# ashvardanian/StringWars

Hardware: AMD Instinct MI355X
Metric: GCUPS (DP cell updates/s) batched Levenshtein (higher is better)
Workload: dtype u32; 1 GPU; C2 tokens64: 1000000 ASCII token pairs per GPU, lengths U[32,96], unbounded Levenshtein, tapes prepared and resident in HBM; step=one synchronous call (results visible on return), pairs_per_gpu=1000000, pairs_total=1000000, cells_per_gpu=4273938131, algorithm=auto, offsets=uint32, collective=none, seed=42

## Files before the change

stringwars_amd/csrc/bp_item.hpp:

```cpp
#pragma once
#include <type_traits>

#include "common.hpp"
#include "bp_window.hpp"

namespace swh {

struct SymWindow32 {
    const uint32_t *base;
    int lo, hi;
    __device__ __forceinline__ void init(const uint32_t *data, uint64_t start, uint64_t total) {
        auto c31 = [](int64_t v) { return (int)(v < -0x40000000ll ? -0x40000000ll : (v > 0x40000000ll ? 0x40000000ll : v)); };
        base = data + start;
        lo = c31(-(int64_t)start);
        hi = c31((int64_t)total - (int64_t)start - 1);
    }
    __device__ __forceinline__ uint32_t fetch(int idx) const { return base[bp_med3i(idx, lo, hi)]; }
    __device__ __forceinline__ void fetch4(int idx, uint32_t (&out)[4]) const {
        if (hi - lo >= 3) {
            const int c = bp_med3i(idx, lo, hi - 3);
            uint4 v;
            __builtin_memcpy(&v, base + c, 16);
            out[0] = v.x; out[1] = v.y; out[2] = v.z; out[3] = v.w;
            if (__builtin_expect(c == idx, 1)) return;
        }
#pragma unroll
        for (int q = 0; q < 4; ++q) out[q] = fetch(idx + q);
    }
};

template <typename Sym> struct BpTraits;
template <> struct BpTraits<uint8_t> {
    static constexpr int kWaves = 4, kEntries = 32, kMinWavesPerSimd = 4;
};
template <> struct BpTraits<uint32_t> {
    static constexpr int kWaves = 2, kEntries = 56, kMinWavesPerSimd = 2;
};
template <typename Sym> constexpr int bp_table_words() { return BpTraits<Sym>::kEntries * 64; }
template <typename Sym> constexpr size_t bp_lds_bytes() {
    return (size_t)BpTraits<Sym>::kWaves * (bp_table_words<Sym>() + 64) * 4 + 80 * 4;
}

struct GroupTables3 {
    uint32_t tbase, mask;
    __device__ __forceinline__ void init(uint32_t *table, int lane) {
        tbase = (uint32_t)(uintptr_t)(lds_u32 *)(table + lane);
        if (tbase & 0x700u) __builtin_trap();
        mask = 0x700u;
        asm volatile("" : "+v"(mask));
    }
    template <int G> __device__ __forceinline__ uint32_t addr(uint32_t c) const {
        uint32_t s;
        if constexpr (3 * G <= 8) s = c << (8 - 3 * G);
        else s = c >> (3 * G - 8);
        return (uint32_t)__builtin_amdgcn_bitop3_b32((int)s, (int)mask, (int)tbase, 0xEA);
    }
    __device__ __forceinline__ uint32_t lookup(uint32_t c) const { return lookup_n<7>(c); }
    __device__ __forceinline__ void insert(uint32_t c, uint32_t bit) const { insert_n<7>(c, bit); }
    template <int NG, int G> __device__ __forceinline__ uint32_t entry_n(uint32_t c) const {
        if constexpr (G + 1 == NG && NG < 7) {
            uint32_t idx = c >> (3 * G);
            idx = idx < 8u ? idx : 8u;
            return *(const lds_u32 *)(uintptr_t)(tbase + (idx << 8) + 2048u * G);
        } else {
            return *(const lds_u32 *)(uintptr_t)(addr<G>(c) + 2048u * G);
        }
    }
    template <int NG> __device__ __forceinline__ uint32_t lookup_n(uint32_t c) const {
        uint32_t e = entry_n<NG, 0>(c) & entry_n<NG, 1>(c);
        e &= entry_n<NG, 2>(c) & entry_n<NG, 3>(c);
        if constexpr (NG > 4) e &= entry_n<NG, 4>(c);
        if constexpr (NG > 5) e &= entry_n<NG, 5>(c);
        if constexpr (NG > 6) e &= entry_n<NG, 6>(c);
        return e;
    }
    template <int NG> __device__ __forceinline__ void insert_n(uint32_t c, uint32_t bit) const {
        __hip_atomic_fetch_or((lds_u32 *)(uintptr_t)addr<0>(c), bit, __ATOMIC_RELAXED, __HIP_MEMORY_SCOPE_WORKGROUP);
        __hip_atomic_fetch_or((lds_u32 *)(uintptr_t)(addr<1>(c) + 2048), bit, __ATOMIC_RELAXED, __HIP_MEMORY_SCOPE_WORKGROUP);
        __hip_atomic_fetch_or((lds_u32 *)(uintptr_t)(addr<2>(c) + 4096), bit, __ATOMIC_RELAXED, __HIP_MEMORY_SCOPE_WORKGROUP);
        __hip_atomic_fetch_or((lds_u32 *)(uintptr_t)(addr<3>(c) + 6144), bit, __ATOMIC_RELAXED, __HIP_MEMORY_SCOPE_WORKGROUP);
        if constexpr (NG > 4) __hip_atomic_fetch_or((lds_u32 *)(uintptr_t)(addr<4>(c) + 8192), bit, __ATOMIC_RELAXED, __HIP_MEMORY_SCOPE_WORKGROUP);
        if constexpr (NG > 5) __hip_atomic_fetch_or((lds_u32 *)(uintptr_t)(addr<5>(c) + 10240), bit, __ATOMIC_RELAXED, __HIP_MEMORY_SCOPE_WORKGROUP);
        if constexpr (NG > 6) __hip_atomic_fetch_or((lds_u32 *)(uintptr_t)(addr<6>(c) + 12288), bit, __ATOMIC_RELAXED, __HIP_MEMORY_SCOPE_WORKGROUP);
    }
};

template <typename Sym>
struct BpWave {
    static constexpr bool kBytes = sizeof(Sym) == 1;
    uint32_t *table;
    uint32_t *acc;
    NibbleTables nib;
    GroupTables3 grp;
    int lane;
    uint64_t a_total, b_total;
    __device__ __forceinline__ void init(uint32_t *table_, uint32_t *acc_, int lane_, uint64_t a_total_, uint64_t b_total_) {
        table = table_; acc = acc_; lane = lane_; a_total = a_total_; b_total = b_total_;
        if constexpr (kBytes) nib.init(table, lane);
        else grp.init(table, lane);
#pragma unroll
        for (int k = 0; k < BpTraits<Sym>::kEntries; ++k) table[k * 64 + lane] = 0;
    }
};

template <typename Sym, bool kWide>
__device__ __forceinline__ void bp_item(const KernelArgs &args, BpWave<Sym> &wv, const uint32_t G, const bool have, const uint64_t p,
                                        const uint64_t a0, const uint32_t la, const uint64_t b0, const uint32_t lb,
                                        uint16_t *staged = nullptr, const uint64_t staged_base = 0) {
    constexpr bool kBytes = sizeof(Sym) == 1;
    constexpr bool wide_tapes = kWide;
    const int lane = wv.lane;
    uint32_t *const table = wv.table;
    uint32_t *const acc = wv.acc;
    [[maybe_unused]] const NibbleTables &nib = wv.nib;
    [[maybe_unused]] const GroupTables3 &grp = wv.grp;
    const uint64_t a_total = wv.a_total, b_total = wv.b_total;
    const uint32_t slot = (uint32_t)lane / G, blk = (uint32_t)lane - slot * G;
    const bool a_is_pattern = bp_pattern_is_a(la, lb);
    const uint32_t m = a_is_pattern ? la : lb, n = a_is_pattern ? lb : la;
    using Window = typename std::conditional<kBytes, ByteWindow, SymWindow32>::type;
    Window pat, txt;
    pat.init((const Sym *)(a_is_pattern ? args.job.a.data : args.job.b.data), a_is_pattern ? a0 : b0,
             a_is_pattern ? a_total : b_total);
    txt.init((const Sym *)(a_is_pattern ? args.job.b.data : args.job.a.data), a_is_pattern ? b0 : a0,
             a_is_pattern ? b_total : a_total);

    const uint32_t row0 = blk * 32;
    const uint32_t brows = have ? (m > row0 ? (m - row0 < 32 ? m - row0 : 32) : 0) : 0;

    constexpr int kTextRegs = kBytes ? 4 : 16;
    uint32_t tnxt[kTextRegs];
    int tshift[kBytes ? 4 : 1];
    auto fetch_text = [&](int first) {
        if constexpr (kBytes) {
            if (wide_tapes) {
                tshift[0] = txt.fetch16_raw(first, tnxt);
            } else {
#pragma unroll
                for (int q = 0; q < 4; ++q) tnxt[q] = txt.fetch4_raw(first + q * 4, tshift[q]);
            }
        } else {
#pragma unroll
            for (int q = 0; q < 16; q += 4) {
                uint32_t four[4];
                txt.fetch4(first + q, four);
#pragma unroll
                for (int r = 0; r < 4; ++r) tnxt[q + r] = four[r];
            }
        }
    };
    fetch_text(0 - (int)blk);
    [[maybe_unused]] uint32_t groups = 7;

    if constexpr (kBytes) {
        uint32_t praw[8];
        int pshift[8];
        if (wide_tapes) {
            uint32_t half[2][4];
            const int moved0 = pat.fetch16_raw((int)row0, half[0]), moved1 = pat.fetch16_raw((int)row0 + 16, half[1]);
            pat.fix16((int)row0, moved0, half[0]);
            pat.fix16((int)row0 + 16, moved1, half[1]);
#pragma unroll
            for (int q = 0; q < 8; ++q) { praw[q] = half[q >> 2][q & 3]; pshift[q] = 24; }
        } else {
#pragma unroll
            for (int q = 0; q < 8; ++q) praw[q] = pat.fetch4_raw((int)row0 + q * 4, pshift[q]);
        }
        const uint32_t row_mask = brows >= 32 ? 0xFFFFFFFFu : ((1u << brows) - 1u);
#pragma unroll
        for (int q = 0; q < 8; ++q) {
            if (brows > (uint32_t)q * 4) {
                const uint32_t dw = ByteWindow::realign(praw[q], pshift[q]);
                nib.template insert<0>(dw, row_mask & (1u << (q * 4 + 0)));
                nib.template insert<1>(dw, row_mask & (1u << (q * 4 + 1)));
                nib.template insert<2>(dw, row_mask & (1u << (q * 4 + 2)));
                nib.template insert<3>(dw, row_mask & (1u << (q * 4 + 3)));
            }
        }
    } else {
        uint32_t psym[32];
#pragma unroll
        for (int q = 0; q < 32; q += 4) {
            uint32_t four[4];
            pat.fetch4((int)row0 + q, four);
#pragma unroll
            for (int r = 0; r < 4; ++r) psym[q + r] = four[r];
        }
        uint32_t seen = 0;
#pragma unroll
        for (int q = 0; q < 32; ++q) seen |= (uint32_t)q < brows ? psym[q] : 0u;
#pragma unroll
        for (int off = 32; off >= 1; off >>= 1) seen |= (uint32_t)__shfl_xor((int)seen, off);
        groups = seen < (1u << 12) ? 4u : (seen < (1u << 15) ? 5u : (seen < (1u << 18) ? 6u : 7u));
        auto enter = [&](auto ng_tag) {
            constexpr int NG = decltype(ng_tag)::value;
#pragma unroll
            for (int q = 0; q < 32; ++q)
                if ((uint32_t)q < brows) grp.template insert_n<NG>(psym[q], 1u << q);
        };
        if (groups == 4) enter(std::integral_constant<int, 4>{});
        else if (groups == 5) enter(std::integral_constant<int, 5>{});
        else if (groups == 6) enter(std::integral_constant<int, 6>{});
        else enter(std::integral_constant<int, 7>{});
    }
    acc[lane] = 0;
    wave_lds_fence();

    const uint32_t n_eff = wave_max_u32(have ? n + G - 1 : 0);
    const uint32_t steps = (n_eff + 15) & ~15u;

    const bool first_blk = blk == 0;
    uint32_t keep_mask = first_blk ? 0u : 0xFFFFFFFFu, first_ph = first_blk ? 0x80000000u : 0u;
    asm volatile("" : "+v"(keep_mask), "+v"(first_ph));
    uint32_t pv = 0xFFFFFFFFu, mv = 0, ph = 0, mh = 0;
    auto column = [&](uint32_t eq, uint32_t s) {
        uint32_t ph_in = (uint32_t)__builtin_amdgcn_update_dpp(0, (int)ph, 0x138, 0xf, 0xf, true);
        uint32_t mh_in = (uint32_t)__builtin_amdgcn_update_dpp(0, (int)mh, 0x138, 0xf, 0xf, true);
        ph_in = (uint32_t)__builtin_amdgcn_bitop3_b32((int)ph_in, (int)keep_mask, (int)first_ph, 0xEA);
        mh_in = mh_in & keep_mask;
        if (s - blk < n) {
            uint32_t xv = eq | mv;
            eq |= mh_in >> 31;
            uint32_t xh = (((eq & pv) + pv) ^ pv) | eq;
            ph = mv | ~(xh | pv);
            mh = pv & xh;
            uint32_t ph_s = __builtin_amdgcn_alignbit(ph, ph_in, 31);
            uint32_t mh_s = __builtin_amdgcn_alignbit(mh, mh_in, 31);
            pv = mh_s | ~(xv | ph_s);
            mv = ph_s & xv;
        }
    };
    auto columns = [&](auto ng_tag) {
    [[maybe_unused]] constexpr int NG = decltype(ng_tag)::value;
    for (uint32_t s0 = 0; s0 < steps; s0 += 16) {
        uint32_t tcur[kTextRegs];
        if constexpr (kBytes) {
            if (wide_tapes) {
#pragma unroll
                for (int q = 0; q < 4; ++q) tcur[q] = tnxt[q];
                txt.fix16((int)s0 - (int)blk, tshift[0], tcur);
            } else {
#pragma unroll
                for (int q = 0; q < 4; ++q) tcur[q] = ByteWindow::realign(tnxt[q], tshift[q]);
            }
        } else {
#pragma unroll
            for (int q = 0; q < kTextRegs; ++q) tcur[q] = tnxt[q];
        }
        fetch_text((int)s0 + 16 - (int)blk);
#pragma unroll
        for (int q = 0; q < 4; ++q) {
            const uint32_t gs = s0 + q * 4;
            if (gs >= n_eff) break;
            uint32_t eqs[4];
            if constexpr (kBytes) {
                eqs[0] = nib.template lookup<0>(tcur[q]);
                eqs[1] = nib.template lookup<1>(tcur[q]);
                eqs[2] = nib.template lookup<2>(tcur[q]);
                eqs[3] = nib.template lookup<3>(tcur[q]);
            } else {
#pragma unroll
                for (int u = 0; u < 4; ++u) eqs[u] = grp.template lookup_n<NG>(tcur[q * 4 + u]);
            }
#pragma unroll
            for (int u = 0; u < 4; ++u) column(eqs[u], gs + u);
        }
    }
    };
    if constexpr (kBytes) columns(std::integral_constant<int, 7>{});
    else if (groups == 4) columns(std::integral_constant<int, 4>{});
    else if (groups == 5) columns(std::integral_constant<int, 5>{});
    else if (groups == 6) columns(std::integral_constant<int, 6>{});
    else columns(std::integral_constant<int, 7>{});

    const uint32_t mask = brows >= 32 ? 0xFFFFFFFFu : ((1u << brows) - 1u);
    int part = __popc(pv & mask) - __popc(mv & mask);
    if (have && brows) atomicAdd(&acc[slot * G], (uint32_t)part);
    wave_lds_fence();
    if (have && first_blk) {
        uint32_t d = n + acc[lane];
        const uint32_t bounded = clamp_bound(d, args.job.bound);
        if (staged && bounded < 0xFFFFu) staged[p - staged_base] = (uint16_t)bounded;
        else store_result(args.job, p, (int64_t)bounded);
    }
    if constexpr (kBytes) {
#pragma unroll
        for (int k = 0; k < BpTraits<Sym>::kEntries; ++k) table[k * 64 + lane] = 0;
    } else {
#pragma unroll
        for (int k = 0; k < 32; ++k) table[k * 64 + lane] = 0;
        if (groups > 4) {
#pragma unroll
            for (int k = 32; k < BpTraits<Sym>::kEntries; ++k) table[k * 64 + lane] = 0;
        }
    }
    wave_lds_fence();
}

}
```

stringwars_amd/csrc/tiled.hip:

```cpp
#include <cstdio>
#include <cstdlib>

#include "bp_item.hpp"

namespace swh {

constexpr int tile_index_bits(int waves) { return waves >= 16 ? 12 : 11; }
constexpr int tile_max(int waves) { return 1 << tile_index_bits(waves); }
constexpr uint32_t kAffixCap = 16;
constexpr int kTileBuckets = 32;
constexpr int kTileClasses = 64;
constexpr int kTileBins = kTileClasses * kTileBuckets;

template <int kTileMax>
struct TileLds {
    uint32_t sorted[kTileMax];
    uint32_t bins[kTileBins / 2 > kTileMax / 2 ? kTileBins / 2 : kTileMax / 2];
    uint32_t class_count[kTileClasses];
    uint16_t class_thr[kTileClasses];
    uint16_t class_tgt[kTileClasses];
    uint32_t item_prefix[kTileClasses + 1];
    uint32_t wave_sums[16];
    uint32_t ticket;
};
struct TileTail {
    unsigned long long cells, syms;
    uint32_t maxa, maxb, shorts, misfit;
    SummaryLds summary;
};
static_assert(sizeof(TileTail) <= sizeof(uint32_t) * kTileBins / 2, "the tail reuses TileLds::bins");

template <typename Sym, int kWaves> constexpr size_t tiled_lds_bytes() {
    return (size_t)kWaves * (bp_table_words<Sym>() + 64) * 4 + sizeof(TileLds<tile_max(kWaves)>);
}

#ifdef SWH_TILE_PROFILE
__device__ unsigned long long g_tile_phase[8];
__device__ unsigned long long g_tile_span[2048][4];
extern "C" void swh_debug_tile_spans(unsigned long long *out) {
    (void)hipDeviceSynchronize();
    (void)hipMemcpyFromSymbol(out, HIP_SYMBOL(g_tile_span), sizeof(unsigned long long) * 2048 * 4);
}
extern "C" void swh_debug_tile_phases(unsigned long long *out) {
    unsigned long long zero[8] = {};
    (void)hipDeviceSynchronize();
    (void)hipMemcpyFromSymbol(out, HIP_SYMBOL(g_tile_phase), sizeof(zero));
    (void)hipMemcpyToSymbol(HIP_SYMBOL(g_tile_phase), zero, sizeof(zero));
}
#define TILE_STAMP(slot) do { const unsigned long long now__ = __builtin_readcyclecounter(); phase_acc[slot] += now__ - phase_t; phase_t = now__; } while (0)
#else
#define TILE_STAMP(slot) do {} while (0)
#endif

struct TiledArgs {
    KernelArgs k;
    uint32_t tile;
    uint32_t tiles;
    uint32_t shift;
    uint32_t cut_affixes;
    PlanPartial *partials;
    uint32_t *done_counter;
    CallSummary *summary;
};

template <typename Sym, int kWaves, bool kWide>
__device__ __forceinline__ void tiled_run(const TiledArgs &targs, char *smem, const uint64_t a_total, const uint64_t b_total) {
    constexpr int kThreads = kWaves * 64, kTableWords = bp_table_words<Sym>();
    constexpr int kTileMax = tile_max(kWaves), kTileIndexBits = tile_index_bits(kWaves);
    constexpr int kPer = (kTileMax + kThreads - 1) / kThreads;
    const KernelArgs &args = targs.k;
    const int lane = threadIdx.x & 63, wave = threadIdx.x >> 6;
    BpWave<Sym> wv;
    wv.init((uint32_t *)smem + (size_t)wave * kTableWords, (uint32_t *)smem + (size_t)kWaves * kTableWords + wave * 64, lane,
            a_total, b_total);
    TileLds<kTileMax> &tl = *(TileLds<kTileMax> *)(smem + (size_t)kWaves * (kTableWords + 64) * 4);
    unsigned long long cells = 0, syms = 0;
    uint32_t maxa = 0, maxb = 0, shorts = 0, misfit = 0;
#ifdef SWH_TILE_PROFILE
    unsigned long long phase_acc[4] = {0, 0, 0, 0}, phase_t = __builtin_readcyclecounter(), items_done = 0;
    if (threadIdx.x == 0) g_tile_span[blockIdx.x][0] = __builtin_amdgcn_s_memrealtime();
#endif

    for (uint32_t tile = blockIdx.x; tile < targs.tiles; tile += gridDim.x) {
        const uint64_t base = (uint64_t)tile * targs.tile;
        const uint32_t count = (uint32_t)(args.job.pairs - base < targs.tile ? args.job.pairs - base : targs.tile);
        __builtin_amdgcn_s_setprio(3);
        for (int i = threadIdx.x; i < kTileBins / 2; i += kThreads) tl.bins[i] = 0;
        if (threadIdx.x < kTileClasses) tl.class_count[threadIdx.x] = 0;
        if (threadIdx.x == 0) tl.ticket = 0;
        __syncthreads();
        uint32_t cls[kPer], txt[kPer], rank[kPer], affix[kPer];
#ifndef SWH_TILE_BATCH
#define SWH_TILE_BATCH 2
#endif
        constexpr int kBatch = kPer < SWH_TILE_BATCH ? kPer : SWH_TILE_BATCH;
        static_assert(kPer % kBatch == 0, "pairs per thread come in whole batches");
#pragma unroll
        for (int kb = 0; kb < kPer; kb += kBatch) {
        uint64_t a0s[kBatch], b0s[kBatch];
        uint32_t las[kBatch], lbs[kBatch];
#pragma unroll
        for (int j = 0; j < kBatch; ++j) {
            const int k = kb + j;
            const uint64_t p = base + (uint32_t)k * kThreads + threadIdx.x;
            const uint64_t pc = p < args.job.pairs ? p : args.job.pairs - 1;
            if (args.off64) pair_extent<uint64_t, true>(args.job, pc, a0s[j], las[j], b0s[j], lbs[j]);
            else pair_extent<uint32_t, true>(args.job, pc, a0s[j], las[j], b0s[j], lbs[j]);
            affix[k] = 0;
        }
        if constexpr (sizeof(Sym) == 1 && kWide) {
            if (targs.cut_affixes) {
                uint4 ha[kBatch], hb[kBatch], ta[kBatch], tb[kBatch];
                bool inside[kBatch];
#pragma unroll
                for (int j = 0; j < kBatch; ++j) {
                    const uint64_t ea = a0s[j] + las[j], eb = b0s[j] + lbs[j];
                    inside[j] = a0s[j] + 16 <= a_total && b0s[j] + 16 <= b_total && ea >= 16 && eb >= 16;
                    const uint8_t *ad = (const uint8_t *)args.job.a.data, *bd = (const uint8_t *)args.job.b.data;
                    __builtin_memcpy(&ha[j], ad + (inside[j] ? a0s[j] : 0), 16);
                    __builtin_memcpy(&hb[j], bd + (inside[j] ? b0s[j] : 0), 16);
                    __builtin_memcpy(&ta[j], ad + (inside[j] ? ea - 16 : 0), 16);
                    __builtin_memcpy(&tb[j], bd + (inside[j] ? eb - 16 : 0), 16);
                }
#pragma unroll
                for (int j = 0; j < kBatch; ++j) {
                    const uint32_t mn = las[j] < lbs[j] ? las[j] : lbs[j];
                    const unsigned long long h_lo = (unsigned long long)(ha[j].x ^ hb[j].x) | ((unsigned long long)(ha[j].y ^ hb[j].y) << 32);
                    const unsigned long long h_hi = (unsigned long long)(ha[j].z ^ hb[j].z) | ((unsigned long long)(ha[j].w ^ hb[j].w) << 32);
                    const unsigned long long t_lo = (unsigned long long)(ta[j].x ^ tb[j].x) | ((unsigned long long)(ta[j].y ^ tb[j].y) << 32);
                    const unsigned long long t_hi = (unsigned long long)(ta[j].z ^ tb[j].z) | ((unsigned long long)(ta[j].w ^ tb[j].w) << 32);
                    uint32_t pre = h_lo ? (uint32_t)__builtin_ctzll(h_lo) >> 3 : (h_hi ? 8u + ((uint32_t)__builtin_ctzll(h_hi) >> 3) : kAffixCap);
                    pre = pre < mn ? pre : mn;
                    uint32_t suf = t_hi ? (uint32_t)__builtin_clzll(t_hi) >> 3 : (t_lo ? 8u + ((uint32_t)__builtin_clzll(t_lo) >> 3) : kAffixCap);
                    suf = suf < mn - pre ? suf : mn - pre;
                    affix[kb + j] = inside[j] ? pre | (suf << 6) : 0u;
                }
            }
        }
#pragma unroll
        for (int j = 0; j < kBatch; ++j) {
            const int k = kb + j;
            const uint32_t idx = (uint32_t)k * kThreads + threadIdx.x;
            cls[k] = 0xFFu; txt[k] = 0; rank[k] = 0;
            if (idx < count) {
                const uint64_t p = base + idx;
                uint32_t la = las[j], lb = lbs[j];
                cells += (unsigned long long)la * lb;
                syms += (unsigned long long)la + lb;
                maxa = la > maxa ? la : maxa;
                maxb = lb > maxb ? lb : maxb;
                shorts += (la <= 32 && lb <= 32) ? 1u : 0u;
                if ((la | lb) >= kStringLimit) { misfit = 1; continue; }
                const uint32_t diff = la > lb ? la - lb : lb - la;
                const uint32_t shared = (affix[k] & 63u) + (affix[k] >> 6);
                la -= shared; lb -= shared;
                if (la == 0 || lb == 0) {
                    store_result(args.job, p, (int64_t)clamp_bound(la + lb, args.job.bound));
                } else if (args.job.bound != 0xFFFFFFFFu && diff > args.job.bound) {
                    store_result(args.job, p, (int64_t)args.job.bound + 1);
                } else {
                    const bool pattern_is_a = bp_pattern_is_a(la, lb);
                    const uint32_t m = pattern_is_a ? la : lb, n = pattern_is_a ? lb : la;
                    const uint32_t g = (m + 31) >> 5;
                    if (g > (uint32_t)kTileClasses) {
                        misfit = 1;
                    } else {
                        cls[k] = g - 1;
                        txt[k] = n;
                        rank[k] = atomicAdd(&tl.class_count[g - 1], 1u);
                    }
                }
            }
        }
        }
        __syncthreads();
        if (wave == 0) {
            const uint32_t mine = tl.class_count[lane];
            tl.class_thr[lane] = (uint16_t)mine;
            tl.class_tgt[lane] = (uint16_t)lane;
            unsigned long long present = __ballot(mine != 0);
            wave_lds_fence();
            if (lane == 0) {
                uint32_t incoming = 0;
                while (present) {
                    const int c = __builtin_ctzll(present);
                    present &= present - 1;
                    const uint32_t native = tl.class_count[c];
                    uint32_t total = native + incoming;
                    incoming = 0;
                    const uint32_t per = 64u / (uint32_t)(c + 1), rest = total % per;
                    if (rest && present) {
                        const int up = __builtin_ctzll(present);
                        const uint32_t per_up = 64u / (uint32_t)(up + 1);
                        if (rest <= native && 2 * rest <= per_up) {
                            tl.class_thr[c] = (uint16_t)(native - rest);
                            tl.class_tgt[c] = (uint16_t)up;
                            incoming = rest;
                            total -= rest;
                        }
                    }
                    tl.class_count[c] = total;
                }
            }
            wave_lds_fence();
            const uint32_t final_count = tl.class_count[lane], per = 64u / (uint32_t)(lane + 1);
            const uint32_t items = (final_count + per - 1) / per;
            const uint32_t incl = wave_inclusive_sum_u32(items);
            tl.item_prefix[lane] = incl - items;
            if (lane == 63) tl.item_prefix[64] = incl;
        }
        __syncthreads();
        uint32_t key[kPer];
#pragma unroll
        for (int k = 0; k < kPer; ++k) {
            key[k] = 0xFFFFFFFFu;
            if (cls[k] != 0xFFu) {
                uint32_t c = cls[k];
                if (rank[k] >= tl.class_thr[c]) c = tl.class_tgt[c];
                const uint32_t bucket = txt[k] >> targs.shift;
                key[k] = c * kTileBuckets + (bucket < (uint32_t)kTileBuckets - 1 ? bucket : (uint32_t)kTileBuckets - 1);
                const uint32_t old = atomicAdd(&tl.bins[key[k] >> 1], (key[k] & 1u) ? 0x10000u : 1u);
                rank[k] = (key[k] & 1u) ? old >> 16 : old & 0xFFFFu;
            }
        }
        __syncthreads();
        {
            constexpr int kWords = (kTileBins / 2 + kThreads - 1) / kThreads;
            uint32_t words[kWords], sum = 0;
#pragma unroll
            for (int q = 0; q < kWords; ++q) {
                const int at = threadIdx.x * kWords + q;
                words[q] = at < kTileBins / 2 ? tl.bins[at] : 0u;
                sum += (words[q] & 0xFFFFu) + (words[q] >> 16);
            }
            const uint32_t incl = wave_inclusive_sum_u32(sum);
            if (lane == 63) tl.wave_sums[wave] = incl;
            __syncthreads();
            uint32_t run = incl - sum;
            for (int w = 0; w < wave; ++w) run += tl.wave_sums[w];
#pragma unroll
            for (int q = 0; q < kWords; ++q) {
                const uint32_t lo = words[q] & 0xFFFFu, hi = words[q] >> 16;
                const int at = threadIdx.x * kWords + q;
                if (at < kTileBins / 2) tl.bins[at] = run | ((run + lo) << 16);
                run += lo + hi;
            }
        }
        __syncthreads();
#pragma unroll
        for (int k = 0; k < kPer; ++k) {
            if (key[k] != 0xFFFFFFFFu) {
                const uint32_t word = tl.bins[key[k] >> 1];
                const uint32_t start = (key[k] & 1u) ? word >> 16 : word & 0xFFFFu;
                tl.sorted[start + rank[k]] = ((uint32_t)k * kThreads + threadIdx.x) | (affix[k] << kTileIndexBits);
            }
        }
        __syncthreads();
        TILE_STAMP(0);
#ifdef SWH_TILE_PROFILE
        if (threadIdx.x == 0) g_tile_span[blockIdx.x][1] = __builtin_amdgcn_s_memrealtime();
#endif
        if (threadIdx.x < kTileClasses) tl.class_thr[threadIdx.x] = (uint16_t)(tl.bins[(threadIdx.x * kTileBuckets) >> 1] & 0xFFFFu);
        __syncthreads();
        static_assert(sizeof(tl.bins) >= (size_t)kTileMax * 2, "the key counters' space holds a tile's distances as 16-bit slots");
        uint16_t *const staged = (uint16_t *)tl.bins;
        for (int i = threadIdx.x; i < kTileMax / 2; i += kThreads) tl.bins[i] = 0xFFFFFFFFu;
        __syncthreads();
        __builtin_amdgcn_s_setprio(0);
        {
            const uint32_t items_total = tl.item_prefix[64];
            const uint32_t my_prefix = tl.item_prefix[lane];
            for (;;) {
                uint32_t t = 0;
                if (lane == 0) t = __hip_atomic_fetch_add(&tl.ticket, 1u, __ATOMIC_RELAXED, __HIP_MEMORY_SCOPE_WORKGROUP);
                t = (uint32_t)__builtin_amdgcn_readfirstlane((int)t);
                if (t >= items_total) break;
                const uint32_t item = items_total - 1 - t;
                const uint32_t G = (uint32_t)__popcll(__ballot(my_prefix <= item));
                const uint32_t per = 64 / G;
                const uint32_t chunk = item - tl.item_prefix[G - 1];
                const uint32_t cstart = tl.class_thr[G - 1], ccount = tl.class_count[G - 1];
                const uint32_t slot = (uint32_t)lane / G;
                const uint32_t pidx = chunk * per + slot;
                const bool have = slot < per && pidx < ccount;
                uint64_t p = 0, a0 = 0, b0 = 0;
                uint32_t la = 0, lb = 0;
                if (have) {
                    const uint32_t entry = tl.sorted[cstart + pidx];
                    p = base + (entry & (uint32_t)(kTileMax - 1));
                    if (args.off64) pair_extent<uint64_t, true>(args.job, p, a0, la, b0, lb);
                    else pair_extent<uint32_t, true>(args.job, p, a0, la, b0, lb);
                    const uint32_t pre = (entry >> kTileIndexBits) & 63u, both = pre + (entry >> (kTileIndexBits + 6));
                    a0 += pre; b0 += pre; la -= both; lb -= both;
                }
                bp_item<Sym, kWide>(args, wv, G, have, p, a0, la, b0, lb, staged, base);
#ifdef SWH_TILE_PROFILE
                ++items_done;
#endif
            }
        }
        TILE_STAMP(1);
        __syncthreads();
        TILE_STAMP(2);
#ifdef SWH_TILE_PROFILE
        if (threadIdx.x == 0) g_tile_span[blockIdx.x][2] = __builtin_amdgcn_s_memrealtime();
#endif
        for (uint32_t i = threadIdx.x; i < count; i += kThreads) {
            const uint32_t d = staged[i];
            if (d != 0xFFFFu) store_result(args.job, base + i, (int64_t)d);
        }
        __syncthreads();
    }
#ifdef SWH_TILE_PROFILE
    if (threadIdx.x == 0) g_tile_span[blockIdx.x][3] = __builtin_amdgcn_s_memrealtime();
    if (lane == 0) {
        for (int q = 0; q < 3; ++q) atomicAdd(&g_tile_phase[q], phase_acc[q]);
        atomicAdd(&g_tile_phase[3], 1ull);
        atomicAdd(&g_tile_phase[4], items_done);
    }
#endif
    {
        TileTail &tail = *(TileTail *)tl.bins;
        unsigned long long &lcells = tail.cells, &lsyms = tail.syms;
        uint32_t &lmaxa = tail.maxa, &lmaxb = tail.maxb, &lshorts = tail.shorts, &lmisfit = tail.misfit;
        if (threadIdx.x == 0) { lcells = 0; lsyms = 0; lmaxa = 0; lmaxb = 0; lshorts = 0; lmisfit = 0; }
        __syncthreads();
#pragma unroll
        for (int off = 32; off >= 1; off >>= 1) {
            cells += __shfl_xor(cells, off);
            syms += __shfl_xor(syms, off);
            shorts += __shfl_xor(shorts, off);
            misfit |= __shfl_xor(misfit, off);
            const uint32_t oa = __shfl_xor(maxa, off), ob = __shfl_xor(maxb, off);
            maxa = oa > maxa ? oa : maxa;
            maxb = ob > maxb ? ob : maxb;
        }
        if (lane == 0) {
            atomicAdd(&lcells, cells);
            atomicAdd(&lsyms, syms);
            atomicMax(&lmaxa, maxa);
            atomicMax(&lmaxb, maxb);
            atomicAdd(&lshorts, shorts);
            atomicOr(&lmisfit, misfit);
        }
        __syncthreads();
        report_call_summary(PlanPartial{lcells, lsyms, lmaxa, lmaxb, lshorts, lmisfit}, targs.partials, targs.done_counter, targs.summary, tail.summary);
    }
}

template <typename Sym, int kWaves>
__global__ __launch_bounds__(kWaves * 64, BpTraits<Sym>::kMinWavesPerSimd) void k_bitparallel_tiled(TiledArgs targs) {
    extern __shared__ __attribute__((aligned(16))) char smem[];
    const KernelArgs &args = targs.k;
    const uint64_t a_total = tape_total(args.job.a, args.off64);
    const uint64_t b_total = tape_total(args.job.b, args.off64);
    if constexpr (sizeof(Sym) == 1) {
        if (a_total >= 16 && b_total >= 16) tiled_run<Sym, kWaves, true>(targs, smem, a_total, b_total);
        else tiled_run<Sym, kWaves, false>(targs, smem, a_total, b_total);
    } else {
        tiled_run<Sym, kWaves, false>(targs, smem, a_total, b_total);
    }
}

TilePlan plan_tiles(uint64_t pairs, uint32_t slots, uint32_t longest_text, uint32_t kTileMax) {
    TilePlan tp{};
    constexpr uint32_t kTileMin = 256;
    const uint64_t rounds = (pairs + (uint64_t)slots * kTileMax - 1) / ((uint64_t)slots * kTileMax);
    uint64_t tile = (pairs + slots * rounds - 1) / (slots * rounds);
    static const uint32_t forced = [] { const char *e = test_hook("STRINGWARS_AMD_TILE"); return e ? (uint32_t)atoi(e) : 0u; }();
    if (forced) tile = forced;
    if (tile < kTileMin) tile = kTileMin;
    if (tile > (uint64_t)kTileMax) tile = kTileMax;
    tp.tile = (uint32_t)tile;
    tp.tiles = (uint32_t)((pairs + tile - 1) / tile);
    tp.blocks = tp.tiles < slots ? tp.tiles : slots;
    uint32_t shift = 0;
    while (((uint64_t)longest_text >> shift) >= (uint64_t)kTileBuckets) ++shift;
    tp.shift = shift;
    return tp;
}

template <typename Sym, int kWaves>
static void launch_tiled_sym(Scope *scope, const KernelArgs &args, uint64_t pairs, uint32_t longest_text) {
    constexpr size_t lds = tiled_lds_bytes<Sym, kWaves>();
    uint32_t slots = (uint32_t)scope->compute_units * (uint32_t)((160 * 1024) / lds);
    if (slots > (uint32_t)kMaxPartials) slots = kMaxPartials;
    const TilePlan tp = plan_tiles(pairs, slots, longest_text, (uint32_t)tile_max(kWaves));
    TiledArgs t{};
    t.k = args;
    t.k.boundary = nullptr;
    t.tile = tp.tile; t.tiles = tp.tiles; t.shift = tp.shift;
    static const bool no_affix = [] { const char *e = test_hook("STRINGWARS_AMD_AFFIX"); return e && atoi(e) == 0; }();
    t.cut_affixes = sizeof(Sym) == 1 && !no_affix ? 1u : 0u;
    t.partials = scope->plan_partials;
    t.done_counter = scope->done_counter;
    t.summary = scope->summary_target();
    opt_in_dynamic_lds(scope, (const void *)k_bitparallel_tiled<Sym, kWaves>, lds);
    static const bool debug = test_hook("STRINGWARS_AMD_DEBUG") != nullptr;
    if (debug) {
        int per_cu = 0;
        (void)hipOccupancyMaxActiveBlocksPerMultiprocessor(&per_cu, k_bitparallel_tiled<Sym, kWaves>, kWaves * 64, lds);
        fprintf(stderr, "[swh] tiled: pairs %llu tile %u tiles %u blocks %u shift %u lds %zu -> %d workgroups per CU\n",
                (unsigned long long)pairs, tp.tile, tp.tiles, tp.blocks, tp.shift, lds, per_cu);
    }
    StampGuard guard(scope, sizeof(Sym) == 1 ? "bitparallel_tiled" : "bitparallel_tiled_u32");
    hipLaunchKernelGGL((k_bitparallel_tiled<Sym, kWaves>), dim3(tp.blocks), dim3(kWaves * 64), lds, scope->stream, t);
    SWH_HIP_CHECK(hipGetLastError());
}

void launch_bitparallel_tiled(Scope *scope, const KernelArgs &args, uint64_t pairs, uint32_t longest_text) {
    static const int forced = [] { const char *e = test_hook("STRINGWARS_AMD_TILED_WAVES"); return e ? atoi(e) : 0; }();
    if (args.sym_bytes == 4) {
        if (forced == 4) launch_tiled_sym<uint32_t, BpTraits<uint32_t>::kWaves>(scope, args, pairs, longest_text);
        else if (forced == 8) launch_tiled_sym<uint32_t, 8>(scope, args, pairs, longest_text);
        else launch_tiled_sym<uint32_t, 10>(scope, args, pairs, longest_text);
    }
    else if (forced == 4) launch_tiled_sym<uint8_t, 4>(scope, args, pairs, longest_text);
    else if (forced == 8) launch_tiled_sym<uint8_t, 8>(scope, args, pairs, longest_text);
    else if (forced == 16 || (!forced && !scope->async && pairs >= (uint64_t)scope->compute_units * 2048)) launch_tiled_sym<uint8_t, 16>(scope, args, pairs, longest_text);
    else launch_tiled_sym<uint8_t, 8>(scope, args, pairs, longest_text);
}

}
```

Measured before the change: 30770 GCUPS.

## Add interior-tile fast path with unclamped 128-bit loads and specialized plain kernel

```diff
diff --git a/stringwars_amd/csrc/bp_item.hpp b/stringwars_amd/csrc/bp_item.hpp
--- a/stringwars_amd/csrc/bp_item.hpp
+++ b/stringwars_amd/csrc/bp_item.hpp
@@ -103,27 +103,64 @@
     }
 };
 
-template <typename Sym, bool kWide>
+typedef uint32_t bp_u32x4 __attribute__((ext_vector_type(4)));
+typedef bp_u32x4 bp_u32x4_unaligned __attribute__((aligned(1)));
+typedef const __attribute__((address_space(1))) uint8_t *bp_global_bytes;
+__device__ __forceinline__ bp_u32x4 bp_load16(bp_global_bytes base, uint32_t offset) {
+    return *(const __attribute__((address_space(1))) bp_u32x4_unaligned *)(base + offset);
+}
+
+struct BpTileItem {
+    uint32_t slot = 0, blk = 0;
+    bool a_is_pattern = false;
+    bp_global_bytes base = nullptr;
+    uint32_t a_off = 0, b_off = 0;
+    uint32_t a_last = 0, b_last = 0;
+};
+enum BpItemMode { kBpAlone = 0, kBpFromTile = 1, kBpInterior = 2 };
+
+constexpr uint32_t kBpMarginLo = 64, kBpMarginHi = 32;
+static_assert(kBpMarginLo >= 63 && kBpMarginHi >= 31 && kBpMarginHi >= 16, "see the derivation above: 64 lanes per wave, 32-row blocks, 16-byte windows");
+
+template <typename Sym, bool kWide, int kMode = kBpAlone>
 __device__ __forceinline__ void bp_item(const KernelArgs &args, BpWave<Sym> &wv, const uint32_t G, const bool have, const uint64_t p,
                                         const uint64_t a0, const uint32_t la, const uint64_t b0, const uint32_t lb,
-                                        uint16_t *staged = nullptr, const uint64_t staged_base = 0) {
+                                        uint16_t *staged = nullptr, const uint64_t staged_base = 0, const BpTileItem &ti = BpTileItem{}) {
     constexpr bool kBytes = sizeof(Sym) == 1;
     constexpr bool wide_tapes = kWide;
+    constexpr bool kInterior = kMode == kBpInterior;
+    static_assert(!kInterior || (kBytes && kWide), "the interior variant is for byte tapes read with 128-bit loads");
     const int lane = wv.lane;
     uint32_t *const table = wv.table;
     uint32_t *const acc = wv.acc;
     [[maybe_unused]] const NibbleTables &nib = wv.nib;
     [[maybe_unused]] const GroupTables3 &grp = wv.grp;
-    const uint64_t a_total = wv.a_total, b_total = wv.b_total;
-    const uint32_t slot = (uint32_t)lane / G, blk = (uint32_t)lane - slot * G;
-    const bool a_is_pattern = bp_pattern_is_a(la, lb);
+    uint32_t slot, blk;
+    bool a_is_pattern;
+    if constexpr (kMode == kBpAlone) {
+        slot = (uint32_t)lane / G; blk = (uint32_t)lane - slot * G;
+        a_is_pattern = bp_pattern_is_a(la, lb);
+    } else {
+        slot = ti.slot; blk = ti.blk; a_is_pattern = ti.a_is_pattern;
+    }
     const uint32_t m = a_is_pattern ? la : lb, n = a_is_pattern ? lb : la;
     using Window = typename std::conditional<kBytes, ByteWindow, SymWindow32>::type;
-    Window pat, txt;
-    pat.init((const Sym *)(a_is_pattern ? args.job.a.data : args.job.b.data), a_is_pattern ? a0 : b0,
-             a_is_pattern ? a_total : b_total);
-    txt.init((const Sym *)(a_is_pattern ? args.job.b.data : args.job.a.data), a_is_pattern ? b0 : a0,
-             a_is_pattern ? b_total : a_total);
+    [[maybe_unused]] Window pat, txt;
+    [[maybe_unused]] uint32_t pat_off = 0, txt_off = 0, txt_last = 0;
+    if constexpr (kInterior) {
+        const uint32_t oa = (uint32_t)a0 + ti.a_off, ob = (uint32_t)b0 + ti.b_off;
+        const uint32_t pat_last = have ? (a_is_pattern ? ti.a_last : ti.b_last) - 16u : kBpMarginLo;
+        txt_last = have ? (a_is_pattern ? ti.b_last : ti.a_last) : kBpMarginLo;
+        pat_off = (a_is_pattern ? oa : ob) + blk * 32u;
+        pat_off = pat_off < pat_last ? pat_off : pat_last;
+        txt_off = (a_is_pattern ? ob : oa) - blk;
+    } else {
+        const uint64_t a_total = wv.a_total, b_total = wv.b_total;
+        pat.init((const Sym *)(a_is_pattern ? args.job.a.data : args.job.b.data), a_is_pattern ? a0 : b0,
+                 a_is_pattern ? a_total : b_total);
+        txt.init((const Sym *)(a_is_pattern ? args.job.b.data : args.job.a.data), a_is_pattern ? b0 : a0,
+                 a_is_pattern ? b_total : a_total);
+    }
 
     const uint32_t row0 = blk * 32;
     const uint32_t brows = have ? (m > row0 ? (m - row0 < 32 ? m - row0 : 32) : 0) : 0;
@@ -132,7 +169,11 @@
     uint32_t tnxt[kTextRegs];
     int tshift[kBytes ? 4 : 1];
     auto fetch_text = [&](int first) {
-        if constexpr (kBytes) {
+        if constexpr (kInterior) {
+            const uint32_t at = txt_off + (uint32_t)first;
+            const bp_u32x4 v = bp_load16(ti.base, at < txt_last ? at : txt_last);
+            tnxt[0] = v.x; tnxt[1] = v.y; tnxt[2] = v.z; tnxt[3] = v.w;
+        } else if constexpr (kBytes) {
             if (wide_tapes) {
                 tshift[0] = txt.fetch16_raw(first, tnxt);
             } else {
@@ -149,13 +190,19 @@
             }
         }
     };
-    fetch_text(0 - (int)blk);
+    fetch_text(kInterior ? 0 : 0 - (int)blk);
     [[maybe_unused]] uint32_t groups = 7;
 
     if constexpr (kBytes) {
         uint32_t praw[8];
         int pshift[8];
-        if (wide_tapes) {
+        if constexpr (kInterior) {
+            const bp_u32x4 v[2] = {bp_load16(ti.base, pat_off), bp_load16(ti.base, pat_off + 16)};
+#pragma unroll
+            for (int q = 0; q < 2; ++q) { praw[4 * q] = v[q].x; praw[4 * q + 1] = v[q].y; praw[4 * q + 2] = v[q].z; praw[4 * q + 3] = v[q].w; }
+#pragma unroll
+            for (int q = 0; q < 8; ++q) pshift[q] = 24;
+        } else if (wide_tapes) {
             uint32_t half[2][4];
             const int moved0 = pat.fetch16_raw((int)row0, half[0]), moved1 = pat.fetch16_raw((int)row0 + 16, half[1]);
             pat.fix16((int)row0, moved0, half[0]);
@@ -234,7 +281,10 @@
     [[maybe_unused]] constexpr int NG = decltype(ng_tag)::value;
     for (uint32_t s0 = 0; s0 < steps; s0 += 16) {
         uint32_t tcur[kTextRegs];
-        if constexpr (kBytes) {
+        if constexpr (kInterior) {
+#pragma unroll
+            for (int q = 0; q < 4; ++q) tcur[q] = tnxt[q];
+        } else if constexpr (kBytes) {
             if (wide_tapes) {
 #pragma unroll
                 for (int q = 0; q < 4; ++q) tcur[q] = tnxt[q];
@@ -247,7 +297,7 @@
 #pragma unroll
             for (int q = 0; q < kTextRegs; ++q) tcur[q] = tnxt[q];
         }
-        fetch_text((int)s0 + 16 - (int)blk);
+        fetch_text(kInterior ? (int)s0 + 16 : (int)s0 + 16 - (int)blk);
 #pragma unroll
         for (int q = 0; q < 4; ++q) {
             const uint32_t gs = s0 + q * 4;
diff --git a/stringwars_amd/csrc/tiled.hip b/stringwars_amd/csrc/tiled.hip
--- a/stringwars_amd/csrc/tiled.hip
+++ b/stringwars_amd/csrc/tiled.hip
@@ -20,9 +20,23 @@
     uint16_t class_thr[kTileClasses];
     uint16_t class_tgt[kTileClasses];
     uint32_t item_prefix[kTileClasses + 1];
-    uint32_t wave_sums[16];
+    union {
+        uint32_t wave_sums[16];
+        struct { unsigned long long lo_a, hi_a, lo_b, hi_b; } span;
+    };
     uint32_t ticket;
 };
+static_assert(sizeof(TileLds<4096>::span) <= sizeof(TileLds<4096>::wave_sums), "the tile's span borrows the scan's wave sums");
+
+__host__ __device__ constexpr uint32_t lane_over(uint32_t x, uint32_t floor_magic) { return (x * floor_magic + x) >> 16; }
+constexpr bool lane_over_is_exact() {
+    for (uint32_t g = 1; g <= 64; ++g)
+        for (uint32_t x = 0; x <= 64; ++x)
+            if (lane_over(x, 65535u / g) != x / g) return false;
+    return true;
+}
+static_assert(lane_over_is_exact(), "lane / G and 64 / G by multiplication");
+
 struct TileTail {
     unsigned long long cells, syms;
     uint32_t maxa, maxb, shorts, misfit;
@@ -58,17 +72,26 @@
     uint32_t tiles;
     uint32_t shift;
     uint32_t cut_affixes;
+    uint32_t no_interior;
     PlanPartial *partials;
     uint32_t *done_counter;
     CallSummary *summary;
 };
 
-template <typename Sym, int kWaves, bool kWide>
+template <typename Sym, int kWaves, bool kWide, bool kPlain = false>
 __device__ __forceinline__ void tiled_run(const TiledArgs &targs, char *smem, const uint64_t a_total, const uint64_t b_total) {
     constexpr int kThreads = kWaves * 64, kTableWords = bp_table_words<Sym>();
     constexpr int kTileMax = tile_max(kWaves), kTileIndexBits = tile_index_bits(kWaves);
     constexpr int kPer = (kTileMax + kThreads - 1) / kThreads;
-    const KernelArgs &args = targs.k;
+    constexpr bool kInteriorTiles = sizeof(Sym) == 1 && kWide && kWaves >= 8;
+    [[maybe_unused]] KernelArgs shaped;
+    const KernelArgs *shaped_or_sent = &targs.k;
+    if constexpr (kPlain) {
+        shaped = targs.k;
+        shaped.off64 = 0; shaped.job.cross = 0; shaped.job.bound = 0xFFFFFFFFu;
+        shaped_or_sent = &shaped;
+    }
+    const KernelArgs &args = *shaped_or_sent;
     const int lane = threadIdx.x & 63, wave = threadIdx.x >> 6;
     BpWave<Sym> wv;
     wv.init((uint32_t *)smem + (size_t)wave * kTableWords, (uint32_t *)smem + (size_t)kWaves * kTableWords + wave * 64, lane,
@@ -87,9 +110,10 @@
         __builtin_amdgcn_s_setprio(3);
         for (int i = threadIdx.x; i < kTileBins / 2; i += kThreads) tl.bins[i] = 0;
         if (threadIdx.x < kTileClasses) tl.class_count[threadIdx.x] = 0;
-        if (threadIdx.x == 0) tl.ticket = 0;
+        if (threadIdx.x == 0) { tl.ticket = 0; tl.span.lo_a = tl.span.lo_b = ~0ull; tl.span.hi_a = tl.span.hi_b = 0; }
         __syncthreads();
         uint32_t cls[kPer], txt[kPer], rank[kPer], affix[kPer];
+        [[maybe_unused]] unsigned long long lo_a = ~0ull, hi_a = 0, lo_b = ~0ull, hi_b = 0;
 #ifndef SWH_TILE_BATCH
 #define SWH_TILE_BATCH 2
 #endif
@@ -145,6 +169,10 @@
             if (idx < count) {
                 const uint64_t p = base + idx;
                 uint32_t la = las[j], lb = lbs[j];
+                if constexpr (kInteriorTiles) {
+                    lo_a = a0s[j] < lo_a ? a0s[j] : lo_a; hi_a = a0s[j] + la > hi_a ? a0s[j] + la : hi_a;
+                    lo_b = b0s[j] < lo_b ? b0s[j] : lo_b; hi_b = b0s[j] + lb > hi_b ? b0s[j] + lb : hi_b;
+                }
                 cells += (unsigned long long)la * lb;
                 syms += (unsigned long long)la + lb;
                 maxa = la > maxa ? la : maxa;
@@ -167,13 +195,50 @@
                     } else {
                         cls[k] = g - 1;
                         txt[k] = n;
+                        affix[k] |= pattern_is_a ? 1u << 12 : 0u;
                         rank[k] = atomicAdd(&tl.class_count[g - 1], 1u);
                     }
                 }
             }
         }
         }
-        __syncthreads();
+        if constexpr (kInteriorTiles) {
+            if (!args.off64) {
+                lo_a = (uint32_t)~wave_max_u32(~(uint32_t)lo_a); hi_a = wave_max_u32((uint32_t)hi_a);
+                lo_b = (uint32_t)~wave_max_u32(~(uint32_t)lo_b); hi_b = wave_max_u32((uint32_t)hi_b);
+            } else {
+#pragma unroll
+                for (int off = 32; off >= 1; off >>= 1) {
+                    const unsigned long long la_ = __shfl_xor(lo_a, off), ha_ = __shfl_xor(hi_a, off), lb_ = __shfl_xor(lo_b, off), hb_ = __shfl_xor(hi_b, off);
+                    lo_a = la_ < lo_a ? la_ : lo_a; hi_a = ha_ > hi_a ? ha_ : hi_a;
+                    lo_b = lb_ < lo_b ? lb_ : lo_b; hi_b = hb_ > hi_b ? hb_ : hi_b;
+                }
+            }
+            if (lane == 0) {
+                atomicMin(&tl.span.lo_a, lo_a); atomicMax(&tl.span.hi_a, hi_a);
+                atomicMin(&tl.span.lo_b, lo_b); atomicMax(&tl.span.hi_b, hi_b);
+            }
+        }
+        __syncthreads();
+        [[maybe_unused]] bool interior = false;
+        [[maybe_unused]] BpTileItem ti;
+        if constexpr (kInteriorTiles) {
+            const unsigned long long s_lo_a = tl.span.lo_a, s_hi_a = tl.span.hi_a, s_lo_b = tl.span.lo_b, s_hi_b = tl.span.hi_b;
+            const bool inside = !targs.no_interior && s_lo_a <= s_hi_a && s_lo_b <= s_hi_b && s_lo_a >= kBpMarginLo && s_lo_b >= kBpMarginLo &&
+                                s_hi_a <= a_total && s_hi_b <= b_total && a_total - s_hi_a >= kBpMarginHi && b_total - s_hi_b >= kBpMarginHi;
+            const unsigned long long da = (unsigned long long)(uintptr_t)args.job.a.data, db = (unsigned long long)(uintptr_t)args.job.b.data;
+            const unsigned long long low = (da + s_lo_a < db + s_lo_b ? da + s_lo_a : db + s_lo_b) - kBpMarginLo;
+            const unsigned long long top = (da + s_hi_a > db + s_hi_b ? da + s_hi_a : db + s_hi_b) + kBpMarginHi;
+            interior = __builtin_amdgcn_readfirstlane((int)(inside && top - low <= (1ull << 31))) != 0;
+            if (interior) {
+                const uint32_t base_lo = (uint32_t)__builtin_amdgcn_readfirstlane((int)(uint32_t)low), base_hi = (uint32_t)__builtin_amdgcn_readfirstlane((int)(uint32_t)(low >> 32));
+                ti.base = (bp_global_bytes)(uintptr_t)(((unsigned long long)base_hi << 32) | base_lo);
+                ti.a_off = (uint32_t)__builtin_amdgcn_readfirstlane((int)(uint32_t)(da - low));
+                ti.b_off = (uint32_t)__builtin_amdgcn_readfirstlane((int)(uint32_t)(db - low));
+                ti.a_last = (uint32_t)__builtin_amdgcn_readfirstlane((int)(uint32_t)(da + s_hi_a + kBpMarginHi - 16 - low));
+                ti.b_last = (uint32_t)__builtin_amdgcn_readfirstlane((int)(uint32_t)(db + s_hi_b + kBpMarginHi - 16 - low));
+            }
+        }
         if (wave == 0) {
             const uint32_t mine = tl.class_count[lane];
             tl.class_thr[lane] = (uint16_t)mine;
@@ -260,14 +325,18 @@
 #ifdef SWH_TILE_PROFILE
         if (threadIdx.x == 0) g_tile_span[blockIdx.x][1] = __builtin_amdgcn_s_memrealtime();
 #endif
-        if (threadIdx.x < kTileClasses) tl.class_thr[threadIdx.x] = (uint16_t)(tl.bins[(threadIdx.x * kTileBuckets) >> 1] & 0xFFFFu);
+        if (threadIdx.x < kTileClasses) {
+            tl.class_thr[threadIdx.x] = (uint16_t)(tl.bins[(threadIdx.x * kTileBuckets) >> 1] & 0xFFFFu);
+            tl.class_tgt[threadIdx.x] = (uint16_t)(65535u / (threadIdx.x + 1u));
+        }
         __syncthreads();
         static_assert(sizeof(tl.bins) >= (size_t)kTileMax * 2, "the key counters' space holds a tile's distances as 16-bit slots");
         uint16_t *const staged = (uint16_t *)tl.bins;
         for (int i = threadIdx.x; i < kTileMax / 2; i += kThreads) tl.bins[i] = 0xFFFFFFFFu;
         __syncthreads();
         __builtin_amdgcn_s_setprio(0);
-        {
+        auto run_items = [&](auto mode_tag) {
+            constexpr int kMode = decltype(mode_tag)::value;
             const uint32_t items_total = tl.item_prefix[64];
             const uint32_t my_prefix = tl.item_prefix[lane];
             for (;;) {
@@ -277,27 +346,39 @@
                 if (t >= items_total) break;
                 const uint32_t item = items_total - 1 - t;
                 const uint32_t G = (uint32_t)__popcll(__ballot(my_prefix <= item));
-                const uint32_t per = 64 / G;
+                const uint32_t over_g = (uint32_t)__builtin_amdgcn_readfirstlane((int)(uint32_t)tl.class_tgt[G - 1]);
+                const uint32_t per = lane_over(64, over_g);
                 const uint32_t chunk = item - tl.item_prefix[G - 1];
                 const uint32_t cstart = tl.class_thr[G - 1], ccount = tl.class_count[G - 1];
-                const uint32_t slot = (uint32_t)lane / G;
+                const uint32_t slot = lane_over((uint32_t)lane, over_g);
                 const uint32_t pidx = chunk * per + slot;
                 const bool have = slot < per && pidx < ccount;
                 uint64_t p = 0, a0 = 0, b0 = 0;
                 uint32_t la = 0, lb = 0;
+                BpTileItem mine = ti;
+                mine.slot = slot; mine.blk = (uint32_t)lane - slot * G;
                 if (have) {
                     const uint32_t entry = tl.sorted[cstart + pidx];
                     p = base + (entry & (uint32_t)(kTileMax - 1));
                     if (args.off64) pair_extent<uint64_t, true>(args.job, p, a0, la, b0, lb);
                     else pair_extent<uint32_t, true>(args.job, p, a0, la, b0, lb);
-                    const uint32_t pre = (entry >> kTileIndexBits) & 63u, both = pre + (entry >> (kTileIndexBits + 6));
+                    const uint32_t pre = (entry >> kTileIndexBits) & 63u, both = pre + ((entry >> (kTileIndexBits + 6)) & 63u);
                     a0 += pre; b0 += pre; la -= both; lb -= both;
-                }
-                bp_item<Sym, kWide>(args, wv, G, have, p, a0, la, b0, lb, staged, base);
+                    mine.a_is_pattern = (entry >> (kTileIndexBits + 12)) & 1u;
+                }
+                bp_item<Sym, kWide, kMode>(args, wv, G, have, p, a0, la, b0, lb, staged, base, mine);
 #ifdef SWH_TILE_PROFILE
                 ++items_done;
 #endif
             }
+        };
+        if constexpr (kInteriorTiles) {
+            if (interior) run_items(std::integral_constant<int, kBpInterior>{});
+            else run_items(std::integral_constant<int, kBpFromTile>{});
+        } else if constexpr (sizeof(Sym) == 1) {
+            run_items(std::integral_constant<int, kBpFromTile>{});
+        } else {
+            run_items(std::integral_constant<int, kBpAlone>{});
         }
         TILE_STAMP(1);
         __syncthreads();
@@ -348,17 +429,17 @@
     }
 }
 
-template <typename Sym, int kWaves>
+template <typename Sym, int kWaves, bool kPlain = false>
 __global__ __launch_bounds__(kWaves * 64, BpTraits<Sym>::kMinWavesPerSimd) void k_bitparallel_tiled(TiledArgs targs) {
     extern __shared__ __attribute__((aligned(16))) char smem[];
     const KernelArgs &args = targs.k;
     const uint64_t a_total = tape_total(args.job.a, args.off64);
     const uint64_t b_total = tape_total(args.job.b, args.off64);
     if constexpr (sizeof(Sym) == 1) {
-        if (a_total >= 16 && b_total >= 16) tiled_run<Sym, kWaves, true>(targs, smem, a_total, b_total);
-        else tiled_run<Sym, kWaves, false>(targs, smem, a_total, b_total);
+        if (a_total >= 16 && b_total >= 16) tiled_run<Sym, kWaves, true, kPlain>(targs, smem, a_total, b_total);
+        else tiled_run<Sym, kWaves, false, kPlain>(targs, smem, a_total, b_total);
     } else {
-        tiled_run<Sym, kWaves, false>(targs, smem, a_total, b_total);
+        tiled_run<Sym, kWaves, false, kPlain>(targs, smem, a_total, b_total);
     }
 }
 
@@ -392,19 +473,25 @@
     t.tile = tp.tile; t.tiles = tp.tiles; t.shift = tp.shift;
     static const bool no_affix = [] { const char *e = test_hook("STRINGWARS_AMD_AFFIX"); return e && atoi(e) == 0; }();
     t.cut_affixes = sizeof(Sym) == 1 && !no_affix ? 1u : 0u;
+    static const bool no_interior = [] { const char *e = test_hook("STRINGWARS_AMD_INTERIOR"); return e && atoi(e) == 0; }();
+    t.no_interior = no_interior ? 1u : 0u;
     t.partials = scope->plan_partials;
     t.done_counter = scope->done_counter;
     t.summary = scope->summary_target();
-    opt_in_dynamic_lds(scope, (const void *)k_bitparallel_tiled<Sym, kWaves>, lds);
+    void (*kernel)(TiledArgs) = k_bitparallel_tiled<Sym, kWaves>;
+    if constexpr (sizeof(Sym) == 1 && kWaves == 16) {
+        if (!args.off64 && !args.job.cross && args.job.bound == 0xFFFFFFFFu) kernel = k_bitparallel_tiled<Sym, kWaves, true>;
+    }
+    opt_in_dynamic_lds(scope, (const void *)kernel, lds);
     static const bool debug = test_hook("STRINGWARS_AMD_DEBUG") != nullptr;
     if (debug) {
         int per_cu = 0;
-        (void)hipOccupancyMaxActiveBlocksPerMultiprocessor(&per_cu, k_bitparallel_tiled<Sym, kWaves>, kWaves * 64, lds);
+        (void)hipOccupancyMaxActiveBlocksPerMultiprocessor(&per_cu, kernel, kWaves * 64, lds);
         fprintf(stderr, "[swh] tiled: pairs %llu tile %u tiles %u blocks %u shift %u lds %zu -> %d workgroups per CU\n",
                 (unsigned long long)pairs, tp.tile, tp.tiles, tp.blocks, tp.shift, lds, per_cu);
     }
     StampGuard guard(scope, sizeof(Sym) == 1 ? "bitparallel_tiled" : "bitparallel_tiled_u32");
-    hipLaunchKernelGGL((k_bitparallel_tiled<Sym, kWaves>), dim3(tp.blocks), dim3(kWaves * 64), lds, scope->stream, t);
+    hipLaunchKernelGGL(kernel, dim3(tp.blocks), dim3(kWaves * 64), lds, scope->stream, t);
     SWH_HIP_CHECK(hipGetLastError());
 }
 
```

Result: faster. 31600 GCUPS, median of 6 (+2.7%).
